# adamjorr/kbbq

Hardware: AMD Instinct MI355X
Metric: recalibrated Gbases/sec (higher is better)
Workload: dtype u64

## Files before the change

kbbq_amd/csrc/bucket.h:

```cpp
#pragma once
#include <hip/hip_runtime.h>
#include <stdint.h>

#include "device_common.h"

namespace kbbq {

constexpr int SUB_BITS = 12;
constexpr int NB2_BITS = 9;
constexpr int SUB_BLOCKS = 1 << SUB_BITS;
constexpr int NB2 = 1 << NB2_BITS;
constexpr int L1_SHIFT = SUB_BITS + NB2_BITS;
constexpr int MAX_NB1 = 512;
constexpr int N_XCD = 8;
constexpr int CNT_STRIDE = 32;
constexpr int BK_THREADS = 512;
constexpr int EMIT_GRID = 512;

struct BucketDev {
    unsigned long long *l1;
    uint32_t *l1_cnt;
    uint32_t *l2;
    uint32_t *l2_cnt;
    uint32_t *tickets;
    unsigned long long *direct;
    uint32_t cap1, cap2;
    int nb1;
    int n_src;
    int cnt_stride;
    uint32_t n_sub;
};

__device__ __forceinline__ int xcc_id() {
    unsigned x;
    asm volatile("s_getreg_b32 %0, hwreg(HW_REG_XCC_ID, 0, 4)" : "=s"(x));
    return (int)(x & (N_XCD - 1));
}

__device__ __forceinline__ uint32_t block_scan512(uint32_t v, uint32_t *wave_tot, uint32_t *total) {
    const int lane = threadIdx.x & 63, w = threadIdx.x >> 6;
    uint32_t inc = v;
#pragma unroll
    for (int o = 1; o < 64; o <<= 1) { const uint32_t y = __shfl_up(inc, o); if (lane >= o) inc += y; }
    if (lane == 63) wave_tot[w] = inc;
    __syncthreads();
    uint32_t before = 0, all = 0;
#pragma unroll
    for (int i = 0; i < 8; ++i) { const uint32_t t = wave_tot[i]; before += i < w ? t : 0; all += t; }
    *total = all;
    return before + inc - v;
}

template <int NW, int CH, bool BY_BASE, int RPW, bool PRIV, bool DENSE = true>
__global__ void __launch_bounds__(BK_THREADS) k_emit_marked(ReadsDev R, KParams K, FiltDev F, BucketDev B, const uint64_t *mask,
                                                             uint64_t mask_words, const uint64_t *kofs,
                                                             unsigned long long *inserted) {
    using S = Stage<NW>;
    constexpr int SLOTS = RPW * CH;
    extern __shared__ unsigned long long sorted[];
    __shared__ uint32_t stage[8][DENSE ? RPW : 1][2 * S::WORDS];
    __shared__ uint32_t hist[MAX_NB1], ofs_l[MAX_NB1], gbase_l[MAX_NB1], fill_l[MAX_NB1], wave_tot[8];
    const int lane = threadIdx.x & 63;
    const int w = __builtin_amdgcn_readfirstlane(threadIdx.x >> 6);
    uint32_t *L32 = stage[w][0];
    const int k = K.k;
    const int src = PRIV ? (int)blockIdx.x : xcc_id();
    const uint64_t reads_per_tile = 8 * RPW;
    const uint64_t n_tiles = (R.n_reads + reads_per_tile - 1) / reads_per_tile;
    unsigned long long mine = 0, direct = 0;
    hist[threadIdx.x] = 0;
    if (PRIV) fill_l[threadIdx.x] = (int)threadIdx.x < B.nb1 ? B.l1_cnt[(size_t)src * B.nb1 + threadIdx.x] : 0u;
    __syncthreads();
    uint64_t off[RPW], kb[RPW], word[RPW];
    uint32_t len[RPW];
    auto fetch_tile = [&](uint64_t tile) {
        const uint64_t r0 = (tile * 8 + w) * RPW;
#pragma unroll
        for (int rr = 0; rr < RPW; ++rr) {
            off[rr] = 0; kb[rr] = 0; word[rr] = 0; len[rr] = 0;
            if (r0 + rr < R.n_reads) {
                read_span(R, r0 + rr, off[rr], len[rr]);
                kb[rr] = BY_BASE ? off[rr] : kmer_base(kofs, r0 + rr, R.read_len, k);
                word[rr] = stage_fetch<NW>(R, nullptr, mask, kb[rr], mask_words - 1, off[rr], lane);
            }
        }
    };
    if (blockIdx.x < n_tiles) fetch_tile(blockIdx.x);
    for (uint64_t tile = blockIdx.x; tile < n_tiles; tile += gridDim.x) {
        unsigned long long rec[SLOTS];
        int rk[SLOTS];
#pragma unroll
        for (int s = 0; s < SLOTS; ++s) { rec[s] = 0; rk[s] = -1; }
        if (DENSE) {
            unsigned long long *wlist = sorted + (size_t)w * SLOTS * 64;
            int n_dense = 0;
            __builtin_amdgcn_wave_barrier();
            if (lane < S::WORDS) {
#pragma unroll
                for (int rr = 0; rr < RPW; ++rr) stage_store(stage[w][rr], lane, word[rr]);
            }
            __builtin_amdgcn_wave_barrier();
#pragma unroll
            for (int rr = 0; rr < RPW; ++rr) {
                const int nk = (int)len[rr] - k + 1;
                if (nk > 0) {
                    const uint32_t *L32 = stage[w][rr];
// ... 27 lines not shown
        } else {
#pragma unroll
        for (int rr = 0; rr < RPW; ++rr) {
            const int nk = (int)len[rr] - k + 1;
            if (nk > 0) {
                __builtin_amdgcn_wave_barrier();
                if (lane < S::WORDS) stage_store(L32, lane, word[rr]);
                __builtin_amdgcn_wave_barrier();
                const int o31 = (int)(off[rr] & 31), o63 = (int)(off[rr] & 63), x63 = (int)(kb[rr] & 63);
#pragma unroll
                for (int c = 0; c < CH; ++c) {
                    if (c * 64 < nk) {
                        const int s = c * 64 + lane;
                        const bool marked = lds_bit(L32 + 2 * S::X, x63 + s) != 0;
                        const bool valid = (lds_window32(L32 + 2 * S::M, o63 + s) & K.nmask_bits) == 0;
                        const bool take = s < nk && marked && (BY_BASE || valid);
                        const uint64_t key = canon_key(lds_window64(L32 + 2 * S::B, 2 * (o31 + s)), K);
                        const uint32_t blk = block_of(F, key);
                        rec[rr * CH + c] = ((unsigned long long)blk << 16) | pattern_of(F, key);
                        if (take) rk[rr * CH + c] = (int)atomicAdd(&hist[blk >> L1_SHIFT], 1u);
                        const unsigned long long bal = __ballot(take);
                        if (!BY_BASE && R.hint_sampled) or_bits64(R.hint_sampled, off[rr] + (uint64_t)c * 64, bal, lane);
                        mine += __popcll(bal);
                    }
                }
            }
        }
        }
        if (tile + gridDim.x < n_tiles) fetch_tile(tile + gridDim.x);
        __syncthreads();
        const uint32_t cnt = hist[threadIdx.x];
        hist[threadIdx.x] = 0;
        uint32_t g = 0;
        if (PRIV) {
            g = fill_l[threadIdx.x];
            fill_l[threadIdx.x] = g + cnt;
        } else if (cnt) {
            g = atomicAdd(&B.l1_cnt[((size_t)src * B.nb1 + threadIdx.x) * CNT_STRIDE], cnt);
        }
        uint32_t total;
        const uint32_t ex = block_scan512(cnt, wave_tot, &total);
        ofs_l[threadIdx.x] = ex;
        gbase_l[threadIdx.x] = g;
        __syncthreads();
#pragma unroll
        for (int s = 0; s < SLOTS; ++s)
            if (rk[s] >= 0) sorted[ofs_l[(uint32_t)(rec[s] >> (16 + L1_SHIFT))] + (uint32_t)rk[s]] = rec[s];
        __syncthreads();
        for (uint32_t i = threadIdx.x; i < total; i += BK_THREADS) {
            const unsigned long long v = sorted[i];
            const uint32_t b = (uint32_t)(v >> (16 + L1_SHIFT));
            const uint32_t pos = gbase_l[b] + (i - ofs_l[b]);
            if (pos < B.cap1) {
                B.l1[((size_t)src * B.nb1 + b) * B.cap1 + pos] = v;
            } else {
                bloom_put(F, (uint32_t)(v >> 16), (uint32_t)(v & 0xFFFFu));
                ++direct;
            }
        }
        if (DENSE) __syncthreads();
    }
    if (PRIV && (int)threadIdx.x < B.nb1) B.l1_cnt[(size_t)src * B.nb1 + threadIdx.x] = fill_l[threadIdx.x];
    if (inserted && lane == 0 && mine) atomicAdd(inserted, mine);
    if (direct) atomicAdd(B.direct, direct);
}

constexpr int SPLIT_PER_THREAD = 12;
constexpr int SPLIT_TILE = BK_THREADS * SPLIT_PER_THREAD;

__global__ void __launch_bounds__(BK_THREADS) k_split(FiltDev F, BucketDev B, uint32_t chunks_per_region) {
    __shared__ uint32_t hist[NB2], ofs_l[NB2], gbase_l[NB2], wave_tot[8], unit_l;
    __shared__ uint32_t sorted[SPLIT_TILE];
    __shared__ uint16_t sorted_b[SPLIT_TILE];
    const int home = xcc_id();
    unsigned long long direct = 0;
    hist[threadIdx.x] = 0;
    for (int qi = 0; qi < N_XCD; ++qi) {
        const int q = (home + qi) & (N_XCD - 1);
        const uint32_t n_buckets = B.nb1 > q ? (uint32_t)(B.nb1 - q + N_XCD - 1) / N_XCD : 0;
        const uint32_t n_units = n_buckets * (uint32_t)B.n_src * chunks_per_region;
        for (;;) {
            __syncthreads();
            if (threadIdx.x == 0) unit_l = atomicAdd(&B.tickets[q * CNT_STRIDE], 1u);
            __syncthreads();
            const uint32_t unit = unit_l;
            if (unit >= n_units) break;
            const uint32_t chunk = unit % chunks_per_region, rest = unit / chunks_per_region;
            const int x = (int)(rest % (uint32_t)B.n_src), b1 = q + (int)(rest / (uint32_t)B.n_src) * N_XCD;
            const size_t region = (size_t)x * B.nb1 + b1;
            const uint32_t n = min(B.l1_cnt[region * B.cnt_stride], B.cap1);
            const uint32_t first = chunk * (uint32_t)SPLIT_TILE;
            if (first >= n) continue;
            const uint32_t m = min((uint32_t)SPLIT_TILE, n - first);
            const unsigned long long *src = B.l1 + region * B.cap1 + first;
            uint32_t rec[SPLIT_PER_THREAD];
            int rk[SPLIT_PER_THREAD];
#pragma unroll
            for (int j = 0; j < SPLIT_PER_THREAD; ++j) {
                const uint32_t i = j * BK_THREADS + threadIdx.x;
                rk[j] = -1;
                rec[j] = 0;
                if (i < m) {
                    const unsigned long long v = src[i];
                    rec[j] = (uint32_t)v;
                    rk[j] = (int)atomicAdd(&hist[(uint32_t)(v >> (16 + SUB_BITS)) & (NB2 - 1)], 1u);
                    rk[j] |= (int)(((uint32_t)(v >> (16 + SUB_BITS)) & (NB2 - 1)) << 16);
                }
            }
            __syncthreads();
            const uint32_t cnt = hist[threadIdx.x];
            hist[threadIdx.x] = 0;
            uint32_t g = 0;
            if (cnt) g = atomicAdd(&B.l2_cnt[(size_t)b1 * NB2 + threadIdx.x], cnt);
            uint32_t total;
            const uint32_t ex = block_scan512(cnt, wave_tot, &total);
            ofs_l[threadIdx.x] = ex;
            gbase_l[threadIdx.x] = g;
            __syncthreads();
#pragma unroll
            for (int j = 0; j < SPLIT_PER_THREAD; ++j)
                if (rk[j] >= 0) {
                    const uint32_t b2 = (uint32_t)rk[j] >> 16, at = ofs_l[b2] + ((uint32_t)rk[j] & 0xFFFFu);
                    sorted[at] = rec[j] & 0x0FFFFFFFu;
                    sorted_b[at] = (uint16_t)b2;
                }
            __syncthreads();
            for (uint32_t i = threadIdx.x; i < total; i += BK_THREADS) {
                const uint32_t v = sorted[i], b2 = sorted_b[i];
                const uint32_t pos = gbase_l[b2] + (i - ofs_l[b2]);
                const size_t sub = (size_t)b1 * NB2 + b2;
                if (pos < B.cap2) {
                    B.l2[sub * B.cap2 + pos] = v;
                } else {
                    bloom_put(F, (uint32_t)(sub << SUB_BITS) | (v >> 16), v & 0xFFFFu);
                    ++direct;
                }
            }
        }
    }
    if (direct) atomicAdd(B.direct, direct);
}

constexpr int APPLY_THREADS = 1024;

__global__ void __launch_bounds__(APPLY_THREADS) k_apply(FiltDev F, BucketDev B) {
    __shared__ ulonglong2 blk_l[SUB_BLOCKS];
    const uint32_t sub = blockIdx.x;
    const uint32_t n = min(B.l2_cnt[sub], B.cap2);
    if (n == 0) return;
    const uint64_t b0 = (uint64_t)sub << SUB_BITS;
    const uint32_t nblk = (uint32_t)min((uint64_t)SUB_BLOCKS, F.n_blocks - b0);
    const uint32_t *src = B.l2 + (size_t)sub * B.cap2;
    const uint32_t last = n - 1;
    uint32_t v[3][4];
    ulonglong2 p[3][4];
#pragma unroll
    for (int s = 0; s < 3; ++s)
#pragma unroll
        for (int j = 0; j < 4; ++j) v[s][j] = src[min(threadIdx.x + (4 * s + j) * APPLY_THREADS, last)];
#pragma unroll
    for (int j = 0; j < 4; ++j) p[0][j] = F.patterns[v[0][j] & 0xFFFFu];
    for (uint32_t i = threadIdx.x; i < nblk; i += APPLY_THREADS) blk_l[i] = F.table[b0 + i];
    __syncthreads();
    unsigned long long *w = reinterpret_cast<unsigned long long *>(blk_l);
    for (uint32_t i1 = threadIdx.x; i1 < n; i1 += 12 * APPLY_THREADS) {
#pragma unroll
        for (int s = 0; s < 3; ++s) {
            const uint32_t i0 = i1 + 4 * s * APPLY_THREADS;
            const int s2 = (s + 1) % 3;
#pragma unroll
            for (int j = 0; j < 4; ++j) p[s2][j] = F.patterns[v[s2][j] & 0xFFFFu];
#pragma unroll
            for (int j = 0; j < 4; ++j) {
                if (i0 + j * APPLY_THREADS < n) {
                    const uint32_t bi = v[s][j] >> 16;
                    const ulonglong2 t = blk_l[bi];
                    const unsigned long long mx = p[s][j].x & ~t.x, my = p[s][j].y & ~t.y;
                    if (mx) atomicOr(&w[2 * bi], mx);
                    if (my) atomicOr(&w[2 * bi + 1], my);
                }
            }
#pragma unroll
            for (int j = 0; j < 4; ++j) v[s][j] = src[min(i0 + (12 + j) * APPLY_THREADS, last)];
        }
    }
    __syncthreads();
    for (uint32_t i = threadIdx.x; i < nblk; i += APPLY_THREADS) F.table[b0 + i] = blk_l[i];
}

}
```

kbbq_amd/csrc/engine.hip:

```cpp
#include <hip/hip_runtime.h>

#include <algorithm>
#include <climits>
#include <cstdarg>
#include <cstdio>
#include <cstdlib>
#include <cstring>
#include <map>
#include <mutex>
#include <string>
#include <thread>
#include <vector>

#include "../../include/kbbq_engine.h"
#include "abi_internal.h"
#include "correct.h"
#include "correct_wave.h"
#include "device_common.h"
#include "host_model.h"

using namespace kbbq;

static thread_local char g_err[512] = "";
int kbbq_fail(int code, const char *fmt, ...) {
// ... 9 lines not shown
        hipError_t _e = (expr);                                                                        \
        if (_e != hipSuccess)                                                                          \
            return fail(_e == hipErrorOutOfMemory ? KBBQ_ENOMEM : KBBQ_EIO, "%s: %s (%s:%d)", #expr,   \
                        hipGetErrorString(_e), __FILE__, __LINE__);                                    \
    } while (0)

#include "kernels.h"
#include "bucket.h"
#include "long_reads.h"


struct FilterHost {
    FilterSpec spec;
    uint64_t *d_table = nullptr;
    uint64_t *d_patterns = nullptr;
    unsigned long long *d_inserted = nullptr;
    uint64_t table_bytes() const { return spec.n_blocks * kEngineBlockBytes; }
    FiltDev dev() const {
        FiltDev f;
        f.table = reinterpret_cast<ulonglong2 *>(d_table);
        f.patterns = reinterpret_cast<const ulonglong2 *>(d_patterns);
        f.n_blocks = spec.n_blocks;
        const ModMagic mm = make_mod_magic(spec.n_blocks);
        f.mod_magic = mm.m64;
        f.mod_m32 = mm.m32;
        f.salt0 = spec.salt[0];
        f.salt1 = spec.salt[1];
        return f;
    }
};

struct ProfileSlot {
    std::string name;
    uint64_t launches = 0;
    double ms = 0;
};
struct PendingEvent {
    int slot;
    hipEvent_t a, b;
};

constexpr int kNoOverride = INT_MIN;
struct Options {
    bool no_overlap = false;
    bool no_fastpath = false;
    bool lane_walk = false;
    bool no_pass4_pipeline = false;
    int pass2_side = 2;
    bool tally_general = false;
    bool infer_subset = true;
    bool debug_bucket = false;
    int bucket = -1;
    uint64_t bucket_records = 0;
    uint64_t pass4_piece = 0;
    int scan_blocks = -1;
    int walk_blocks = -1;
    int infer_blocks = 0;
    int subset_edge = kNoOverride;
    int subset_pmask = kNoOverride;
};


enum Scratch {
    S_KMER_PREFIX,
    S_HOST_OUT,
    S_HOST_FLAGS,
    S_DRAW0, S_DRAW1,
    S_TAKE1,
    S_READ_INDEX0, S_READ_INDEX1,
    S_TMASK, S_DIRTY, S_LIST, S_ERR, S_PATCH,
    S_OFFCASE_LIST,
    S_WALK_WORDS,
    S_SIDE1,
    S_COUNT = S_SIDE1 + (S_SIDE1 - S_TMASK),
    S_TAKE0 = S_ERR + (S_SIDE1 - S_TMASK),
};
constexpr int per_side(Scratch name, int side) { return name + side * (S_SIDE1 - S_TMASK); }

struct SideCounters { unsigned long long list_len, queries; };
struct Counters {
    SideCounters side0;
    unsigned long long kmer_total;
    unsigned long long infer_fetched;
    SideCounters side1;
    unsigned long long offcase_len[2];
    SideCounters *side(int s) { return s ? &side1 : &side0; }
};
struct Tickets {
    unsigned int infer, scan[2], walk[2], unused[11];
};
struct Totals {
    unsigned long long walk_reads, walk_queries;
    unsigned long long digest, unused;
};
static_assert(sizeof(Counters) == 64 && offsetof(Counters, kmer_total) == 16 && offsetof(Counters, side1) == 32 && offsetof(Counters, offcase_len) == 48, "d_counters");
static_assert(sizeof(Tickets) == 64 && offsetof(Tickets, scan) == 4 && offsetof(Tickets, walk) == 12, "d_tickets");
static_assert(sizeof(Totals) == 32 && offsetof(Totals, digest) == 16, "d_totals");

struct Pass3 {
    int side;
    hipStream_t stream;
    int stream_no;
    unsigned long long *cnt;
    unsigned int *scan_ticket, *wave_ticket;
    bool shared;
};
// ... 392 lines not shown

int upload_dq(kbbq_engine *e) {
    const DqTables &d = e->dq;
    const size_t nb = d.n_rg * kNQ, nc = d.n_rg * kNQ * 2 * d.n_cycle, nd = d.n_rg * kNQ * 16;
    std::vector<int16_t> base(nb);
    std::vector<int8_t> cyc(nc), di(nd);
    for (uint64_t r = 0; r < d.n_rg; ++r)
        for (int q = 0; q < kNQ; ++q) base[r * kNQ + q] = (int16_t)(d.meanq[r] + d.rgdq[r] + d.qdq[r * kNQ + q]);
    for (size_t i = 0; i < nc; ++i) cyc[i] = (int8_t)d.cycledq[i];
    for (size_t i = 0; i < nd; ++i) di[i] = (int8_t)d.dinucdq[i];
    HIP_TRY(hipMemcpyAsync(e->d_dq_base, base.data(), nb * 2, hipMemcpyHostToDevice, e->stream));
    HIP_TRY(hipMemcpyAsync(e->d_dq_cycle, cyc.data(), nc, hipMemcpyHostToDevice, e->stream));
    HIP_TRY(hipMemcpyAsync(e->d_dq_dinuc, di.data(), nd, hipMemcpyHostToDevice, e->stream));
    uint8_t slot[KBBQ_NQ];
    memset(slot, 255, sizeof slot);
    int n_slots = 0;
    for (int q = 0; q < kNQ; ++q) {
        bool any = false;
        for (uint64_t r = 0; r < d.n_rg && !any; ++r) {
            const size_t c0 = (r * kNQ + q) * 2 * d.n_cycle, d0 = (r * kNQ + q) * 16;
            for (size_t i = 0; i < 2 * d.n_cycle && !any; ++i) any = cyc[c0 + i] != 0;
            for (size_t i = 0; i < 16 && !any; ++i) any = di[d0 + i] != 0;
        }
        if (any && n_slots < 255) slot[q] = (uint8_t)n_slots;
        if (any) ++n_slots;
    }
    e->dq_slots = n_slots;
    HIP_TRY(hipMemcpyAsync(e->d_dq_qslot, slot, KBBQ_NQ, hipMemcpyHostToDevice, e->stream));
    HIP_TRY(hipStreamSynchronize(e->stream));
    e->dq_set = true;
    return KBBQ_OK;
}

uint64_t env_u64(const char *name, uint64_t dflt) {
    const char *v = getenv(name);
    return v && *v ? strtoull(v, nullptr, 10) : dflt;
}

constexpr bool bucket_private() { return true; }

void bucket_shape(uint64_t n_blocks, uint64_t capacity, uint32_t *n_sub, int *nb1, uint32_t *cap1, uint32_t *cap2) {
    *n_sub = (uint32_t)((n_blocks + SUB_BLOCKS - 1) >> SUB_BITS);
    *nb1 = (int)((*n_sub + NB2 - 1) >> NB2_BITS);
    const double f1 = std::min(1.0, (double)(1ULL << L1_SHIFT) / (double)n_blocks), f2 = std::min(1.0, (double)SUB_BLOCKS / (double)n_blocks);
    const int n_src = bucket_private() ? EMIT_GRID : N_XCD;
    *cap1 = (uint32_t)std::min(4.0e9, (double)capacity * 1.15 * f1 / n_src) + 64;
    *cap2 = (uint32_t)std::min(4.0e9, (double)capacity * 1.25 * f2) + 32;
}

BucketDev bucket_dev(kbbq_engine *e, int w) {
    BucketDev B;
    bucket_shape(e->filt[w].spec.n_blocks, e->bk.capacity, &B.n_sub, &B.nb1, &B.cap1, &B.cap2);
    B.l1 = (unsigned long long *)e->bk.l1;
    B.l2 = (uint32_t *)e->bk.l2;
    B.l1_cnt = e->bk.l1_cnt;
    B.l2_cnt = e->bk.l2_cnt;
    B.tickets = e->bk.tickets;
    B.direct = e->bk.direct;
    B.n_src = bucket_private() ? EMIT_GRID : N_XCD;
    B.cnt_stride = bucket_private() ? 1 : CNT_STRIDE;
    return B;
}

const size_t kL1CntBytes = (size_t)EMIT_GRID * MAX_NB1 * 4, kL2CntBytes = (size_t)MAX_NB1 * NB2 * 4, kTicketBytes = (size_t)N_XCD * CNT_STRIDE * 4;

bool bucket_on(kbbq_engine *e, int w) {
    kbbq_engine::Buckets &b = e->bk;
    if (b.mode[w] >= 0) return b.mode[w] == 1;
    const uint64_t n_blocks = e->filt[w].spec.n_blocks;
    bool want = e->opt.bucket >= 0 ? e->opt.bucket != 0 : e->filt[w].table_bytes() >= (256u << 20);
    if (n_blocks > ((uint64_t)MAX_NB1 << L1_SHIFT)) want = false;
    if (want && !b.allocated) {
        size_t free_b = 0, total_b = 0;
        if (hipMemGetInfo(&free_b, &total_b) != hipSuccess) free_b = 0;
        const uint64_t big = std::max(e->filt[0].spec.n_blocks, e->filt[1].spec.n_blocks);
        uint64_t cap = (uint64_t)((double)free_b * 0.45 / 14.5);
        cap = std::min<uint64_t>(cap, 4000000000ULL);
        cap = std::min<uint64_t>(cap, std::max<uint64_t>(1u << 20, 32 * big));
        if (e->opt.bucket_records) cap = e->opt.bucket_records;
        cap = std::max<uint64_t>(cap, 4096);
        size_t l1_bytes = 0, l2_bytes = 0;
        for (int f = 0; f < 2; ++f) {
            uint32_t n_sub, cap1, cap2; int nb1;
            bucket_shape(e->filt[f].spec.n_blocks, cap, &n_sub, &nb1, &cap1, &cap2);
            l1_bytes = std::max(l1_bytes, (size_t)(bucket_private() ? EMIT_GRID : N_XCD) * nb1 * cap1 * 8);
            l2_bytes = std::max(l2_bytes, (size_t)n_sub * cap2 * 4);
        }
        hipError_t he = hipMalloc(&b.l1, l1_bytes);
        if (he == hipSuccess) he = hipMalloc(&b.l2, l2_bytes);
        if (he == hipSuccess) he = hipMalloc(&b.l1_cnt, kL1CntBytes);
        if (he == hipSuccess) he = hipMalloc(&b.l2_cnt, kL2CntBytes);
        if (he == hipSuccess) he = hipMalloc(&b.tickets, kTicketBytes);
        if (he == hipSuccess) he = hipMalloc(&b.direct, 8);
        if (he == hipSuccess) he = hipMemsetAsync(b.l1_cnt, 0, kL1CntBytes, e->stream);
        if (he == hipSuccess) he = hipMemsetAsync(b.l2_cnt, 0, kL2CntBytes, e->stream);
        if (he == hipSuccess) he = hipMemsetAsync(b.direct, 0, 8, e->stream);
        if (he != hipSuccess) {
            (void)hipGetLastError();
            hipFree(b.l1); hipFree(b.l2); hipFree(b.l1_cnt); hipFree(b.l2_cnt); hipFree(b.tickets); hipFree(b.direct);
            b.l1 = b.l2 = nullptr; b.l1_cnt = b.l2_cnt = b.tickets = nullptr; b.direct = nullptr;
            want = false;
            b.mode[0] = b.mode[1] = 0;
        } else {
            b.allocated = true;
            b.capacity = cap;
        }
    }
    if (b.mode[w] < 0) b.mode[w] = want ? 1 : 0;
    return b.mode[w] == 1;
}

hipStream_t bucket_stream(kbbq_engine *e, int w) { return e->bk.stream[w] ? e->bk.stream[w] : e->stream; }

void bucket_poll_estimate(kbbq_engine *e) {
    kbbq_engine::Buckets &b = e->bk;
    if (!b.est_pending || hipEventQuery(b.ev_est) != hipSuccess) return;
    const unsigned long long now = *b.h_inserted;
    if (b.est_bases > 0 && now >= b.est_prev)
        b.frac_trusted = std::min(1.0, 1.03 * (double)(now - b.est_prev) / (double)b.est_bases + 0.005);
    b.inserted_at_flush[1] = now;
    b.est_pending = false;
    if (e->opt.debug_bucket) fprintf(stderr, "[bucket] inserted %llu (before %llu) over %llu bases -> %.4f trusted inserts per base\n", now,
                       (unsigned long long)b.est_prev, (unsigned long long)b.est_bases, b.frac_trusted);
}

int bucket_flush(kbbq_engine *e, int w, bool barrier = true) {
    kbbq_engine::Buckets &b = e->bk;
    if (!b.pending[w]) return KBBQ_OK;
    const BucketDev B = bucket_dev(e, w);
    const FiltDev F = e->filt[w].dev();
    const hipStream_t emit_st = bucket_stream(e, w);
    hipStream_t st = emit_st;
    int rc;
    if (w == 1 && e->opt.pass2_side == 2 && emit_st != e->stream) {
        st = e->stream;
        if ((rc = run_after(st, emit_st, b.ev_flush))) return rc;
    }
    HIP_TRY(hipMemsetAsync(b.tickets, 0, kTicketBytes, st));
    {
        Timed t(e, w ? "k_split_trusted" : "k_split_sampled", st);
        const uint32_t chunks = (B.cap1 + SPLIT_TILE - 1) / SPLIT_TILE;
        hipLaunchKernelGGL(k_split, dim3(256 * 3), dim3(BK_THREADS), 0, st, F, B, chunks);
        HIP_TRY(hipGetLastError());
    }
    {
        Timed t(e, w ? "k_apply_trusted" : "k_apply_sampled", st);
        hipLaunchKernelGGL(k_apply, dim3(B.n_sub), dim3(APPLY_THREADS), 0, st, F, B);
        HIP_TRY(hipGetLastError());
    }
    HIP_TRY(hipMemsetAsync(b.l1_cnt, 0, kL1CntBytes, st));
    HIP_TRY(hipMemsetAsync(b.l2_cnt, 0, (size_t)B.nb1 * NB2 * 4, st));
    if (st != emit_st && (rc = run_after(emit_st, st, b.ev_flush))) return rc;
    if (st != e->stream && barrier && (rc = run_after(e->stream, st, b.ev_flush))) return rc;
    if (w == 1 && !barrier) {
        bucket_poll_estimate(e);
        if (!b.est_pending && b.h_inserted) {
            HIP_TRY(hipMemcpyAsync(b.h_inserted, e->filt[1].d_inserted, 8, hipMemcpyDeviceToHost, e->stream));
            HIP_TRY(hipEventRecord(b.ev_est, e->stream));
            b.est_pending = true;
            b.est_bases = b.bases_since[1] + b.cur_bases;
            b.est_prev = b.inserted_at_flush[1];
            if (!b.est_known) {
                HIP_TRY(hipEventSynchronize(b.ev_est));
                bucket_poll_estimate(e);
                b.est_known = true;
            }
        }
    }
    if (e->opt.debug_bucket) fprintf(stderr, "[bucket] flush %d of filter %d: estimate %.3g records over %llu bases (%.4f per base), barrier %d\n",
                       (int)b.flushes[w], w, b.pending_est[w], (unsigned long long)b.bases_since[w], w ? b.frac_trusted : 0.0, (int)barrier);
    b.bases_since[w] = 0;
    b.pending[w] = false;
    b.pending_est[w] = 0;
    b.flushes[w] += 1;
    return KBBQ_OK;
}

int bucket_flush_all(kbbq_engine *e) {
    for (int w = 0; w < 2; ++w) {
        int rc = bucket_flush(e, w);
        if (rc) return rc;
    }
    return KBBQ_OK;
}

int settle(kbbq_engine *e) {
    int rc = bucket_flush_all(e);
    return rc ? rc : sync_engine(e);
}

int bucket_reserve(kbbq_engine *e, int w, double est, uint64_t bases) {
    kbbq_engine::Buckets &b = e->bk;
    int rc = bucket_flush(e, 1 - w);
    if (rc) return rc;
    b.cur_bases = bases;
    if (b.pending[w] && b.pending_est[w] + est > 0.93 * (double)b.capacity) {
        if ((rc = bucket_flush(e, w, false))) return rc;
        if (w == 1) est = (est - 4096.0) / std::max(1e-9, b.frac_used) * b.frac_trusted + 4096.0;
    }
    b.cur_bases = 0;
    b.pending[w] = true;
    b.pending_est[w] += est;
    b.bases_since[w] += bases;
    return KBBQ_OK;
}

}


extern "C" {

const char *kbbq_last_error(void) { return g_err; }

int kbbq_engine_create(const kbbq_params *params, kbbq_engine **out) {
    if (!params || !out) return fail(KBBQ_EINVAL, "null argument");
    if (params->k < 1 || params->k > KBBQ_MAX_KMER) return fail(KBBQ_ERANGE, "k must be <= %d and > 0", KBBQ_MAX_KMER);
    if (params->n_rg < 1 || params->n_rg > 65535) return fail(KBBQ_EINVAL, "n_rg must be in 1..65535");
    if (params->max_read_len < 1 || params->max_read_len > KBBQ_MAX_READ_LEN)
        return fail(KBBQ_ERANGE, "max_read_len must be in 1..%d", KBBQ_MAX_READ_LEN);
    int ndev = 0;
    if (hipGetDeviceCount(&ndev) != hipSuccess || ndev == 0) return fail(KBBQ_ENODEV, "no HIP device visible");
    if (params->device < 0 || params->device >= ndev) return fail(KBBQ_ENODEV, "device %d of %d", params->device, ndev);
    DeviceGuard create_guard(params->device);
    HIP_TRY(create_guard.err);
    kbbq_engine *e = new kbbq_engine;
    e->p = *params;
    {
        Options &o = e->opt;
        auto env_set = [](const char *name) { const char *v = getenv(name); return v && *v; };
        auto env_int = [](const char *name, int dflt) { const char *v = getenv(name); return v && *v ? atoi(v) : dflt; };
        const int fl = params->flags;
        o.no_overlap = (fl & KBBQ_F_NO_OVERLAP) || env_set("KBBQ_NO_OVERLAP");
        o.no_fastpath = (fl & KBBQ_F_NO_FASTPATH) || env_set("KBBQ_NO_FASTPATH");
        o.lane_walk = (fl & KBBQ_F_LANE_WALK) || (getenv("KBBQ_CORRECT") && !strcmp(getenv("KBBQ_CORRECT"), "lane"));
        o.no_pass4_pipeline = (fl & KBBQ_F_NO_PASS4_PIPELINE) || env_set("KBBQ_NO_PASS4_PIPELINE");
        o.pass2_side = (fl & KBBQ_F_PASS2_INORDER) ? 0 : env_int("KBBQ_PASS2_SIDE", o.pass2_side);
        o.tally_general = env_set("KBBQ_TALLY_GENERAL");
        o.infer_subset = env_int("KBBQ_INFER_SUBSET", 1) != 0;
        o.debug_bucket = env_set("KBBQ_DEBUG_BUCKET");
        o.bucket = (fl & KBBQ_F_BUCKET_ON) ? 1 : (fl & KBBQ_F_BUCKET_OFF) ? 0 : env_set("KBBQ_BUCKET") ? (env_int("KBBQ_BUCKET", 0) != 0 ? 1 : 0) : -1;
        o.bucket_records = env_u64("KBBQ_BUCKET_RECORDS", 0);
        o.pass4_piece = env_u64("KBBQ_PASS4_PIECE", 0);
        o.scan_blocks = env_int("KBBQ_SCAN_BLOCKS", o.scan_blocks);
        o.walk_blocks = env_int("KBBQ_WALK_BLOCKS", o.walk_blocks);
        o.infer_blocks = env_int("KBBQ_INFER_BLOCKS", o.infer_blocks);
        o.subset_edge = env_int("KBBQ_SUBSET_EDGE", o.subset_edge);
        o.subset_pmask = env_int("KBBQ_SUBSET_PMASK", o.subset_pmask);
    }
    e->K.k = params->k;
    e->K.shift = 2u * (unsigned)(params->k - 1);
    e->K.mask = params->k < 32 ? ((1ULL << (2 * params->k)) - 1) : ~0ULL;
    e->K.nmask_bits = params->k < 32 ? ((1u << params->k) - 1) : 0xFFFFFFFFu;
    const double fprs[2] = {params->fpr_sampled, params->fpr_trusted};
    for (int w = 0; w < 2; ++w) {
        if (!make_filter_spec(params->approx_kmers, fprs[w], params->bloom_seed, e->filt[w].spec)) {
            delete e;
            return fail(KBBQ_EINVAL, "Error: Invalid bloom filter parameters. Adjust parameters and try again.");
        }
    }
    hipError_t he = hipStreamCreateWithFlags(&e->stream, hipStreamNonBlocking);
    if (he == hipSuccess) he = hipStreamCreateWithFlags(&e->stream2, hipStreamNonBlocking);
    if (he == hipSuccess) he = hipStreamCreateWithFlags(&e->copy, hipStreamNonBlocking);
    for (hipEvent_t *ev : engine_events(e))
        if (he == hipSuccess) he = hipEventCreateWithFlags(ev, hipEventDisableTiming);
    if (he == hipSuccess) he = hipHostMalloc((void **)&e->bk.h_inserted, 64, hipHostMallocDefault);
    if (he != hipSuccess) { kbbq_engine_destroy(e); return fail(KBBQ_EIO, "hipStreamCreate: %s", hipGetErrorString(he)); }
#define CREATE_TRY(expr)                                                                           \
    do {                                                                                           \
        hipError_t _e = (expr);                                                                    \
        if (_e != hipSuccess) {                                                                    \
            int code = _e == hipErrorOutOfMemory ? KBBQ_ENOMEM : KBBQ_EIO;                         \
            fail(code, "%s: %s", #expr, hipGetErrorString(_e));                                    \
            kbbq_engine_destroy(e);                                                                \
            return code;                                                                           \
        }                                                                                          \
    } while (0)
    CREATE_TRY(hipMalloc(&e->d_counters, sizeof(Counters)));
    CREATE_TRY(hipMemset(e->d_counters, 0, sizeof(Counters)));
    CREATE_TRY(hipMalloc(&e->d_tickets, sizeof(Tickets)));
    CREATE_TRY(hipMemset(e->d_tickets, 0, sizeof(Tickets)));
    CREATE_TRY(hipMalloc(&e->d_totals, sizeof(Totals)));
    CREATE_TRY(hipMemset(e->d_totals, 0, sizeof(Totals)));
    CREATE_TRY(hipMalloc(&e->d_dq_qslot, KBBQ_NQ));
    CREATE_TRY(hipMalloc(&e->d_qpresent, 32));
    for (int i = 0; i < 2; ++i) CREATE_TRY(hipMalloc(&e->d_rg_present[i], (((size_t)params->n_rg + 31) / 32) * 4 + 4));
    for (int w = 0; w < 2; ++w) {
        FilterHost &f = e->filt[w];
        CREATE_TRY(hipMalloc(&f.d_table, f.table_bytes()));
        CREATE_TRY(hipMalloc(&f.d_patterns, kNumPatterns * kEngineBlockBytes));
        CREATE_TRY(hipMalloc(&f.d_inserted, 8));
        std::vector<uint64_t> packed(kNumPatterns * 2);
        for (uint64_t i = 0; i < kNumPatterns; ++i) {
            if (!squeeze_block(&f.spec.patterns[i * 8], &packed[i * 2])) {
                kbbq_engine_destroy(e);
// ... 61 lines not shown
    if (rc0) return rc0;
    for (int w = 0; w < 2; ++w) {
        HIP_TRY(hipMemsetAsync(e->filt[w].d_table, 0, e->filt[w].table_bytes(), e->stream));
        HIP_TRY(hipMemsetAsync(e->filt[w].d_inserted, 0, 8, e->stream));
    }
    HIP_TRY(hipMemsetAsync(e->d_hist, 0, (e->hist_cycle_words + e->hist_dinuc_words) * 8, e->stream));
    HIP_TRY(hipMemsetAsync(e->d_counters, 0, sizeof(Counters), e->stream));
    HIP_TRY(hipMemsetAsync(e->d_totals, 0, offsetof(Totals, digest), e->stream));
    HIP_TRY(hipMemsetAsync(e->d_qpresent, 0, 32, e->stream));
    memset(e->qpresent, 0, sizeof e->qpresent);
    e->qpresent_known = false;
    if (e->bk.allocated) {
        HIP_TRY(hipMemsetAsync(e->bk.l1_cnt, 0, kL1CntBytes, e->stream));
        HIP_TRY(hipMemsetAsync(e->bk.l2_cnt, 0, kL2CntBytes, e->stream));
        HIP_TRY(hipMemsetAsync(e->bk.direct, 0, 8, e->stream));
    }
    e->bk.est_pending = false;
    e->bk.est_known = false;
    e->bk.frac_trusted = 0.75;
    e->bk.stream[0] = e->bk.stream[1] = nullptr;
    for (int w = 0; w < 2; ++w) { e->bk.pending[w] = false; e->bk.pending_est[w] = 0; e->bk.bases_since[w] = 0; e->bk.inserted_at_flush[w] = 0; e->bk.flushes[w] = 0; }
    e->thresholds_set = false;
    e->dq_set = false;
    memset(e->stats, 0, sizeof e->stats);
    return sync_engine(e);
}

int kbbq_engine_sync(kbbq_engine *e) {
    ENGINE_DEVICE(e);
    return settle(e);
}

void *kbbq_engine_stream(kbbq_engine *e) { return e ? (void *)e->stream : nullptr; }

int kbbq_engine_dims(kbbq_engine *e, uint64_t *n_rg, uint64_t *n_cycle) {
    if (!e) return fail(KBBQ_EINVAL, "null engine");
    if (n_rg) *n_rg = (uint64_t)e->p.n_rg;
    if (n_cycle) *n_cycle = (uint64_t)e->p.max_read_len;
    return KBBQ_OK;
}

int kbbq_engine_tune(kbbq_engine *e, const char *name, uint64_t value) {
    if (!e || !name) return fail(KBBQ_EINVAL, "null argument");
    if (!strcmp(name, "bucket_records")) {
        if (e->bk.allocated) return fail(KBBQ_ESTATE, "the record buffers are allocated already");
        e->opt.bucket_records = value;
    } else if (!strcmp(name, "pass4_piece")) {
        e->opt.pass4_piece = value;
    } else if (!strcmp(name, "scan_blocks") || !strcmp(name, "walk_blocks") || !strcmp(name, "infer_blocks")) {
        if (value > 17) return fail(KBBQ_EINVAL, "%s: 0 (as many as fit) to 16 workgroups per CU, 17 = default", name);
        (name[0] == 's' ? e->opt.scan_blocks : name[0] == 'w' ? e->opt.walk_blocks : e->opt.infer_blocks) = value == 17 ? (name[0] == 'i' ? 0 : -1) : (int)value;
    } else if (!strcmp(name, "infer_subset")) {
        e->opt.infer_subset = value != 0;
    } else if (!strcmp(name, "pass2_side") || !strcmp(name, "no_overlap")) {
        ENGINE_DEVICE(e);
        int rc = settle(e);
        if (rc) return rc;
        if (name[0] == 'p' && value > 2) return fail(KBBQ_EINVAL, "pass2_side: 0, 1 or 2");
        if (name[0] == 'p') e->opt.pass2_side = (int)value; else e->opt.no_overlap = value != 0;
        e->bk.stream[0] = e->bk.stream[1] = nullptr;
    } else {
        return fail(KBBQ_EINVAL, "unknown knob '%s'", name);
    }
    return KBBQ_OK;
}

int kbbq_filter_info_get(kbbq_engine *e, int which, kbbq_filter_info *out) {
    ENGINE_DEVICE(e);
    if (!out || which < 0 || which > 1) return fail(KBBQ_EINVAL, "bad argument");
    int rc = settle(e);
    if (rc) return rc;
    const FilterSpec &s = e->filt[which].spec;
    memset(out, 0, sizeof *out);
    out->bits = s.bits;
    out->bits_unblocked = s.bits_unblocked;
    out->n_blocks = s.n_blocks;
    out->table_bytes = e->filt[which].table_bytes();
    out->random_seed = s.random_seed;
    out->n_hash = s.n_hash;
    out->n_salt = s.n_salt;
    for (uint32_t i = 0; i < s.n_salt; ++i) out->salt[i] = s.salt[i];
    HIP_TRY(hipMemcpy(&out->inserted, e->filt[which].d_inserted, 8, hipMemcpyDeviceToHost));
    return KBBQ_OK;
}

void *kbbq_filter_device_table(kbbq_engine *e, int which) {
    if (!e || which < 0 || which > 1) return nullptr;
    DeviceGuard guard(e->p.device);
    if (guard.err != hipSuccess || bucket_flush_all(e) != KBBQ_OK) return nullptr;
    return e->filt[which].d_table;
}
void *kbbq_filter_device_counter(kbbq_engine *e, int which) { return e && which >= 0 && which < 2 ? e->filt[which].d_inserted : nullptr; }

int kbbq_filter_download(kbbq_engine *e, int which, uint64_t *host_words, uint64_t n_words) {
    ENGINE_DEVICE(e);
    if (!host_words || which < 0 || which > 1) return fail(KBBQ_EINVAL, "bad argument");
    const uint64_t n_blocks = e->filt[which].spec.n_blocks;
    if (n_words != n_blocks * 8) return fail(KBBQ_EINVAL, "filter has %llu words", (unsigned long long)n_blocks * 8);
    int rc = settle(e);
    if (rc) return rc;
    const uint64_t chunk = 1 << 20;
    std::vector<uint64_t> packed(chunk * 2);
    for (uint64_t b0 = 0; b0 < n_blocks; b0 += chunk) {
        const uint64_t nb = std::min(chunk, n_blocks - b0);
        HIP_TRY(hipMemcpy(packed.data(), e->filt[which].d_table + b0 * 2, nb * kEngineBlockBytes, hipMemcpyDeviceToHost));
        for (uint64_t b = 0; b < nb; ++b) expand_block(&packed[b * 2], host_words + (b0 + b) * 8);
// ... 398 lines not shown
int kbbq_device_memory(int32_t device, uint64_t *free_bytes, uint64_t *total_bytes) {
    int cur = 0;
    HIP_TRY(hipGetDevice(&cur));
    if (device >= 0 && device != cur) HIP_TRY(hipSetDevice(device));
    size_t f = 0, t = 0;
    HIP_TRY(hipMemGetInfo(&f, &t));
    if (device >= 0 && device != cur) HIP_TRY(hipSetDevice(cur));
    if (free_bytes) *free_bytes = f;
    if (total_bytes) *total_bytes = t;
    return KBBQ_OK;
}

int kbbq_count_kmer_positions(kbbq_engine *e, const kbbq_reads *reads, uint64_t *out) {
    ENGINE_DEVICE(e);
    if (!reads || !out) return fail(KBBQ_EINVAL, "null argument");
    HostBatchDone host_done(e, reads);
    ReadsDev R; int max_len;
    int rc = device_view(e, reads, &R, &max_len, false);
    if (rc) return rc;
    const uint64_t *kofs;
    return kmer_prefix(e, R, &kofs, out);
}

}

constexpr int kStagedMax = 512;
constexpr int kTallyMaxWindows = 24;
template <template <int> class Launcher, typename... Args>
static int dispatch_nw(int max_len, Args... args) {
    if (max_len <= 192) return Launcher<3>::go(args...);
    if (max_len <= 320) return Launcher<5>::go(args...);
    return Launcher<8>::go(args...);
}

template <int NW> struct LaunchSample {
    static int go(kbbq_engine *e, ReadsDev R, const uint64_t *mask, uint64_t mask_words, const uint64_t *kofs) {
        Timed t(e, "k_insert_sampled");
        hipLaunchKernelGGL((k_insert_marked<NW, false>), dim3(wave_grid(R.n_reads)), dim3(256), 0, e->stream, R, e->K,
                           e->filt[0].dev(), mask, mask_words, kofs, e->filt[0].d_inserted);
        HIP_TRY(hipGetLastError());
        return KBBQ_OK;
    }
};

template <int NW, int CH, int RPW>
static int launch_emit(kbbq_engine *e, int w, ReadsDev R, const uint64_t *mask, uint64_t mask_words, const uint64_t *kofs,
                       unsigned long long *inserted) {
    const BucketDev B = bucket_dev(e, w);
    const uint64_t n_tiles = (R.n_reads + 8 * RPW - 1) / (8 * RPW);
    const int grid = (int)std::min<uint64_t>(n_tiles, EMIT_GRID);
    const size_t lds = (size_t)8 * RPW * CH * 64 * 8;
    hipStream_t st = bucket_stream(e, w);
    Timed t(e, w ? "k_emit_trusted" : "k_emit_sampled", st);
#define KBBQ_EMIT(BYB)                                                                                                        \
    do {                                                                                                                      \
        const void *fn = (const void *)k_emit_marked<NW, CH, BYB, RPW, true, true>;                                            \
        size_t &raised = e->attr_lds_correct[fn];                                                                             \
        if (lds > 48 * 1024 && lds > raised) {                                                                                \
            HIP_TRY(hipFuncSetAttribute(fn, hipFuncAttributeMaxDynamicSharedMemorySize, (int)lds));                            \
            raised = lds;                                                                                                     \
        }                                                                                                                     \
        hipLaunchKernelGGL((k_emit_marked<NW, CH, BYB, RPW, true, true>), dim3(grid), dim3(BK_THREADS), lds, st, R, e->K,      \
                           e->filt[w].dev(), B, mask, mask_words, kofs, inserted);                                            \
    } while (0)
    if (w == 0) KBBQ_EMIT(false); else KBBQ_EMIT(true);
#undef KBBQ_EMIT
    HIP_TRY(hipGetLastError());
    return KBBQ_OK;
}

static int dispatch_emit(kbbq_engine *e, int w, int max_len, ReadsDev R, const uint64_t *mask, uint64_t mask_words, const uint64_t *kofs,
                         unsigned long long *inserted) {
    const int max_nk = std::max(1, max_len - e->p.k + 1);
    if (max_len <= 192) {
        if (max_nk <= 128) return launch_emit<3, 2, 4>(e, w, R, mask, mask_words, kofs, inserted);
        return launch_emit<3, 3, 4>(e, w, R, mask, mask_words, kofs, inserted);
    }
    if (max_len <= 320) return launch_emit<5, 5, 2>(e, w, R, mask, mask_words, kofs, inserted);
    return launch_emit<8, 8, 1>(e, w, R, mask, mask_words, kofs, inserted);
}

extern "C" {

int kbbq_sample_batch(kbbq_engine *e, const kbbq_reads *reads, uint64_t first_kmer_ordinal) {
    ENGINE_DEVICE(e);
    HostBatchDone host_done(e, reads);
    ReadsDev R; int max_len;
    int rc = device_view(e, reads, &R, &max_len, false);
    if (rc) return rc;
    const uint64_t *kofs; uint64_t n_draws;
    if ((rc = kmer_prefix(e, R, &kofs, &n_draws))) return rc;
    if (n_draws == 0) return KBBQ_OK;
    const bool overlap = reads->on_device && !e->opt.no_overlap;
    const int turn = overlap ? e->draw_turn : 0;
    uint64_t *mask;
    if ((rc = scratch_buf(e, turn ? S_DRAW1 : S_DRAW0, (n_draws / 64 + 2) * 8, &mask))) return rc;
    hipStream_t ds = overlap ? e->stream2 : e->stream;
    if (overlap) {
        e->draw_turn ^= 1;
        if (e->ins_pending[turn]) HIP_TRY(hipStreamWaitEvent(ds, e->ev_ins[turn], 0));
    }
    {
        Timed t(e, "k_draw_mask", ds);
        const uint64_t lanes = (n_draws + DRAWS_PER_LANE - 1) / DRAWS_PER_LANE;
        uint64_t st[4];
        xoshiro_state_at(e->p.seed, first_kmer_ordinal, st);
        hipLaunchKernelGGL(k_draw_mask, dim3((unsigned)((lanes + 255) / 256)), dim3(256), 0, ds,
                           st[0], st[1], st[2], st[3],
                           (uint64_t)0, n_draws, e->draw_threshold, e->draw_always ? 1 : 0, mask);
        HIP_TRY(hipGetLastError());
    }
    if (overlap && (rc = run_after(e->stream, ds, e->ev_draw))) return rc;
    if (max_len > kStagedMax) {
        Timed t(e, "k_insert_sampled_long");
        hipLaunchKernelGGL(k_insert_marked_long<false>, dim3(wave_grid(R.n_reads)), dim3(256), 0, e->stream, R, e->K, e->filt[0].dev(),
                           (const uint64_t *)mask, n_draws / 64 + 2, kofs, e->filt[0].d_inserted);
        HIP_TRY(hipGetLastError());
        rc = KBBQ_OK;
// ... 849 lines not shown
```

Before: 24.44.

## Prefetch next split tile and add optional narrow L1 record layout

Restructures k_split so ticket fetch and the global load of the next tile's records overlap with the scatter of the current tile, software-pipelining across loop iterations. It also adds an optional split lo/hi (5-byte) L1 record layout, enabled with KBBQ_L1_WIDE=0, which cuts L1 traffic compared with 8-byte records. Wide records stay the default, so only the prefetching restructure runs by default. The pipelining adds register pressure and more complex control flow.

New measurement: 23.73. 2.9% lower.

```diff
diff --git a/kbbq_amd/csrc/bucket.h b/kbbq_amd/csrc/bucket.h
--- a/kbbq_amd/csrc/bucket.h
+++ b/kbbq_amd/csrc/bucket.h
@@ -18,6 +18,8 @@
 constexpr int EMIT_GRID = 512;
 
 struct BucketDev {
+    uint32_t *l1_lo;
+    uint8_t *l1_hi;
     unsigned long long *l1;
     uint32_t *l1_cnt;
     uint32_t *l2;
@@ -51,7 +53,7 @@
     return before + inc - v;
 }
 
-template <int NW, int CH, bool BY_BASE, int RPW, bool PRIV, bool DENSE = true>
+template <int NW, int CH, bool BY_BASE, int RPW, bool PRIV, bool DENSE = true, bool WIDE = false>
 __global__ void __launch_bounds__(BK_THREADS) k_emit_marked(ReadsDev R, KParams K, FiltDev F, BucketDev B, const uint64_t *mask,
                                                              uint64_t mask_words, const uint64_t *kofs,
                                                              unsigned long long *inserted) {
@@ -185,7 +187,13 @@
             const uint32_t b = (uint32_t)(v >> (16 + L1_SHIFT));
             const uint32_t pos = gbase_l[b] + (i - ofs_l[b]);
             if (pos < B.cap1) {
-                B.l1[((size_t)src * B.nb1 + b) * B.cap1 + pos] = v;
+                const size_t at = ((size_t)src * B.nb1 + b) * B.cap1 + pos;
+                if (WIDE) {
+                    B.l1[at] = v;
+                } else {
+                    B.l1_lo[at] = (uint32_t)v;
+                    B.l1_hi[at] = (uint8_t)((uint32_t)(v >> 32) & 31u);
+                }
             } else {
                 bloom_put(F, (uint32_t)(v >> 16), (uint32_t)(v & 0xFFFFu));
                 ++direct;
@@ -199,65 +207,99 @@
 }
 
 constexpr int SPLIT_PER_THREAD = 12;
+constexpr uint32_t SPLIT_DONE = 0xFFFFFFFFu;
 constexpr int SPLIT_TILE = BK_THREADS * SPLIT_PER_THREAD;
 
+template <bool WIDE>
 __global__ void __launch_bounds__(BK_THREADS) k_split(FiltDev F, BucketDev B, uint32_t chunks_per_region) {
-    __shared__ uint32_t hist[NB2], ofs_l[NB2], gbase_l[NB2], wave_tot[8], unit_l;
-    __shared__ uint32_t sorted[SPLIT_TILE];
-    __shared__ uint16_t sorted_b[SPLIT_TILE];
+    constexpr int SPT = SPLIT_PER_THREAD, TILE = SPLIT_TILE;
+    static_assert(TILE <= 0x10000, "ranks are kept in 16 bits");
+    __shared__ uint32_t hist[NB2], ofs_l[NB2], gbase_l[NB2], wave_tot[8], unit_l[2][4];
+    __shared__ uint32_t sorted[TILE];
+    __shared__ uint16_t sorted_b[TILE];
     const int home = xcc_id();
-    unsigned long long direct = 0;
+    uint32_t direct = 0;
     hist[threadIdx.x] = 0;
-    for (int qi = 0; qi < N_XCD; ++qi) {
-        const int q = (home + qi) & (N_XCD - 1);
-        const uint32_t n_buckets = B.nb1 > q ? (uint32_t)(B.nb1 - q + N_XCD - 1) / N_XCD : 0;
-        const uint32_t n_units = n_buckets * (uint32_t)B.n_src * chunks_per_region;
-        for (;;) {
-            __syncthreads();
-            if (threadIdx.x == 0) unit_l = atomicAdd(&B.tickets[q * CNT_STRIDE], 1u);
-            __syncthreads();
-            const uint32_t unit = unit_l;
-            if (unit >= n_units) break;
-            const uint32_t chunk = unit % chunks_per_region, rest = unit / chunks_per_region;
-            const int x = (int)(rest % (uint32_t)B.n_src), b1 = q + (int)(rest / (uint32_t)B.n_src) * N_XCD;
-            const size_t region = (size_t)x * B.nb1 + b1;
-            const uint32_t n = min(B.l1_cnt[region * B.cnt_stride], B.cap1);
-            const uint32_t first = chunk * (uint32_t)SPLIT_TILE;
-            if (first >= n) continue;
-            const uint32_t m = min((uint32_t)SPLIT_TILE, n - first);
-            const unsigned long long *src = B.l1 + region * B.cap1 + first;
-            uint32_t rec[SPLIT_PER_THREAD];
-            int rk[SPLIT_PER_THREAD];
-#pragma unroll
-            for (int j = 0; j < SPLIT_PER_THREAD; ++j) {
-                const uint32_t i = j * BK_THREADS + threadIdx.x;
-                rk[j] = -1;
-                rec[j] = 0;
-                if (i < m) {
-                    const unsigned long long v = src[i];
-                    rec[j] = (uint32_t)v;
-                    rk[j] = (int)atomicAdd(&hist[(uint32_t)(v >> (16 + SUB_BITS)) & (NB2 - 1)], 1u);
-                    rk[j] |= (int)(((uint32_t)(v >> (16 + SUB_BITS)) & (NB2 - 1)) << 16);
-                }
-            }
-            __syncthreads();
+    int tq = 0;
+    uint32_t ticket = 0;
+    if (threadIdx.x == 0) ticket = atomicAdd(&B.tickets[home * CNT_STRIDE], 1u);
+    uint32_t b1 = 0, m = 0, b1_n = 0, m_n = 0;
+    size_t at_n = 0;
+    uint32_t lo[SPT], hi[SPT];
+#pragma unroll
+    for (int j = 0; j < SPT; ++j) lo[j] = hi[j] = 0;
+    auto load_next = [&]() {
+        if (m_n == 0) return;
+        const uint32_t last = m_n - 1;
+#pragma unroll
+        for (int j = 0; j < SPT; ++j) {
+            const uint32_t i = min(j * BK_THREADS + threadIdx.x, last);
+            if (WIDE) {
+                const unsigned long long v = (B.l1 + at_n)[i];
+                lo[j] = (uint32_t)v;
+                hi[j] = (uint32_t)(v >> 32);
+            } else {
+                lo[j] = (B.l1_lo + at_n)[i];
+                hi[j] = (B.l1_hi + at_n)[i];
+            }
+        }
+    };
+    for (uint32_t it = 0;; ++it) {
+        if (b1 == SPLIT_DONE) break;
+        if (threadIdx.x == 0) {
+            uint32_t pb1 = SPLIT_DONE, pregion = 0, pfirst = 0;
+            while (tq < N_XCD) {
+                const int q = (home + tq) & (N_XCD - 1);
+                const uint32_t n_buckets = B.nb1 > q ? (uint32_t)(B.nb1 - q + N_XCD - 1) / N_XCD : 0;
+                const uint32_t n_units = n_buckets * (uint32_t)B.n_src * chunks_per_region;
+                if (ticket < n_units) {
+                    const uint32_t chunk = ticket % chunks_per_region, rest = ticket / chunks_per_region;
+                    pb1 = (uint32_t)q + (rest / (uint32_t)B.n_src) * N_XCD;
+                    pregion = (rest % (uint32_t)B.n_src) * (uint32_t)B.nb1 + pb1;
+                    pfirst = chunk * (uint32_t)TILE;
+                    break;
+                }
+                if (++tq < N_XCD) ticket = atomicAdd(&B.tickets[((home + tq) & (N_XCD - 1)) * CNT_STRIDE], 1u);
+            }
+            uint32_t *u = unit_l[it & 1];
+            u[0] = pb1; u[1] = pregion; u[2] = pfirst;
+            if (tq < N_XCD) ticket = atomicAdd(&B.tickets[((home + tq) & (N_XCD - 1)) * CNT_STRIDE], 1u);
+        }
+        if (m) {
+#pragma unroll
+            for (int j = 0; j < SPT; ++j) {
+                const uint32_t b2 = ((hi[j] << 4) | (lo[j] >> 28)) & (NB2 - 1);
+                hi[j] = SPLIT_DONE;
+                if (j * BK_THREADS + threadIdx.x < m) hi[j] = atomicAdd(&hist[b2], 1u) | (b2 << 16);
+            }
+        }
+        __syncthreads();
+        const uint32_t *u = unit_l[it & 1];
+        const uint32_t region_v = u[1];
+        const uint32_t b1_f = __builtin_amdgcn_readfirstlane(u[0]), first_f = __builtin_amdgcn_readfirstlane(u[2]);
+        uint32_t n_f = 0;
+        if (b1_f != SPLIT_DONE) n_f = B.l1_cnt[(size_t)region_v * B.cnt_stride];
+        uint32_t total = 0;
+        if (m) {
             const uint32_t cnt = hist[threadIdx.x];
             hist[threadIdx.x] = 0;
             uint32_t g = 0;
             if (cnt) g = atomicAdd(&B.l2_cnt[(size_t)b1 * NB2 + threadIdx.x], cnt);
-            uint32_t total;
             const uint32_t ex = block_scan512(cnt, wave_tot, &total);
             ofs_l[threadIdx.x] = ex;
             gbase_l[threadIdx.x] = g;
             __syncthreads();
 #pragma unroll
-            for (int j = 0; j < SPLIT_PER_THREAD; ++j)
-                if (rk[j] >= 0) {
-                    const uint32_t b2 = (uint32_t)rk[j] >> 16, at = ofs_l[b2] + ((uint32_t)rk[j] & 0xFFFFu);
-                    sorted[at] = rec[j] & 0x0FFFFFFFu;
+            for (int j = 0; j < SPT; ++j)
+                if (hi[j] != SPLIT_DONE) {
+                    const uint32_t b2 = hi[j] >> 16, at = ofs_l[b2] + (hi[j] & 0xFFFFu);
+                    sorted[at] = lo[j] & 0x0FFFFFFFu;
                     sorted_b[at] = (uint16_t)b2;
                 }
             __syncthreads();
+        }
+        load_next();
+        if (m) {
             for (uint32_t i = threadIdx.x; i < total; i += BK_THREADS) {
                 const uint32_t v = sorted[i], b2 = sorted_b[i];
                 const uint32_t pos = gbase_l[b2] + (i - ofs_l[b2]);
@@ -270,8 +312,14 @@
                 }
             }
         }
+        b1 = b1_n;
+        m = m_n;
+        b1_n = b1_f;
+        const uint32_t n = min((uint32_t)__builtin_amdgcn_readfirstlane(n_f), B.cap1);
+        m_n = b1_n != SPLIT_DONE && first_f < n ? min((uint32_t)TILE, n - first_f) : 0u;
+        at_n = (size_t)__builtin_amdgcn_readfirstlane(region_v) * B.cap1 + first_f;
     }
-    if (direct) atomicAdd(B.direct, direct);
+    if (direct) atomicAdd(B.direct, (unsigned long long)direct);
 }
 
 constexpr int APPLY_THREADS = 1024;
diff --git a/kbbq_amd/csrc/engine.hip b/kbbq_amd/csrc/engine.hip
--- a/kbbq_amd/csrc/engine.hip
+++ b/kbbq_amd/csrc/engine.hip
@@ -85,6 +85,7 @@
     bool debug_bucket = false;
     int bucket = -1;
     uint64_t bucket_records = 0;
+    bool l1_wide = true;
     uint64_t pass4_piece = 0;
     int scan_blocks = -1;
     int walk_blocks = -1;
@@ -583,6 +584,8 @@
     BucketDev B;
     bucket_shape(e->filt[w].spec.n_blocks, e->bk.capacity, &B.n_sub, &B.nb1, &B.cap1, &B.cap2);
     B.l1 = (unsigned long long *)e->bk.l1;
+    B.l1_lo = (uint32_t *)e->bk.l1;
+    B.l1_hi = (uint8_t *)e->bk.l1 + (size_t)(bucket_private() ? EMIT_GRID : N_XCD) * B.nb1 * B.cap1 * 4;
     B.l2 = (uint32_t *)e->bk.l2;
     B.l1_cnt = e->bk.l1_cnt;
     B.l2_cnt = e->bk.l2_cnt;
@@ -671,7 +674,8 @@
     {
         Timed t(e, w ? "k_split_trusted" : "k_split_sampled", st);
         const uint32_t chunks = (B.cap1 + SPLIT_TILE - 1) / SPLIT_TILE;
-        hipLaunchKernelGGL(k_split, dim3(256 * 3), dim3(BK_THREADS), 0, st, F, B, chunks);
+        if (e->opt.l1_wide) hipLaunchKernelGGL(k_split<true>, dim3(256 * 3), dim3(BK_THREADS), 0, st, F, B, chunks);
+        else hipLaunchKernelGGL(k_split<false>, dim3(256 * 3), dim3(BK_THREADS), 0, st, F, B, chunks);
         HIP_TRY(hipGetLastError());
     }
     {
@@ -771,6 +775,7 @@
         o.debug_bucket = env_set("KBBQ_DEBUG_BUCKET");
         o.bucket = (fl & KBBQ_F_BUCKET_ON) ? 1 : (fl & KBBQ_F_BUCKET_OFF) ? 0 : env_set("KBBQ_BUCKET") ? (env_int("KBBQ_BUCKET", 0) != 0 ? 1 : 0) : -1;
         o.bucket_records = env_u64("KBBQ_BUCKET_RECORDS", 0);
+        o.l1_wide = env_int("KBBQ_L1_WIDE", 1) != 0;
         o.pass4_piece = env_u64("KBBQ_PASS4_PIECE", 0);
         o.scan_blocks = env_int("KBBQ_SCAN_BLOCKS", o.scan_blocks);
         o.walk_blocks = env_int("KBBQ_WALK_BLOCKS", o.walk_blocks);
@@ -938,6 +943,12 @@
         (name[0] == 's' ? e->opt.scan_blocks : name[0] == 'w' ? e->opt.walk_blocks : e->opt.infer_blocks) = value == 17 ? (name[0] == 'i' ? 0 : -1) : (int)value;
     } else if (!strcmp(name, "infer_subset")) {
         e->opt.infer_subset = value != 0;
+    } else if (!strcmp(name, "l1_wide")) {
+        if (e->bk.pending[0] || e->bk.pending[1]) return fail(KBBQ_ESTATE, "l1_wide: records are pending (kbbq_engine_sync first)");
+        ENGINE_DEVICE(e);
+        int rc = settle(e);
+        if (rc) return rc;
+        e->opt.l1_wide = value != 0;
     } else if (!strcmp(name, "pass2_side") || !strcmp(name, "no_overlap")) {
         ENGINE_DEVICE(e);
         int rc = settle(e);
@@ -1442,18 +1453,19 @@
     const size_t lds = (size_t)8 * RPW * CH * 64 * 8;
     hipStream_t st = bucket_stream(e, w);
     Timed t(e, w ? "k_emit_trusted" : "k_emit_sampled", st);
-#define KBBQ_EMIT(BYB)                                                                                                        \
+#define KBBQ_EMIT(BYB, WIDE)                                                                                                  \
     do {                                                                                                                      \
-        const void *fn = (const void *)k_emit_marked<NW, CH, BYB, RPW, true, true>;                                            \
+        const void *fn = (const void *)k_emit_marked<NW, CH, BYB, RPW, true, true, WIDE>;                                      \
         size_t &raised = e->attr_lds_correct[fn];                                                                             \
         if (lds > 48 * 1024 && lds > raised) {                                                                                \
             HIP_TRY(hipFuncSetAttribute(fn, hipFuncAttributeMaxDynamicSharedMemorySize, (int)lds));                            \
             raised = lds;                                                                                                     \
         }                                                                                                                     \
-        hipLaunchKernelGGL((k_emit_marked<NW, CH, BYB, RPW, true, true>), dim3(grid), dim3(BK_THREADS), lds, st, R, e->K,      \
+        hipLaunchKernelGGL((k_emit_marked<NW, CH, BYB, RPW, true, true, WIDE>), dim3(grid), dim3(BK_THREADS), lds, st, R, e->K, \
                            e->filt[w].dev(), B, mask, mask_words, kofs, inserted);                                            \
     } while (0)
-    if (w == 0) KBBQ_EMIT(false); else KBBQ_EMIT(true);
+    if (e->opt.l1_wide) { if (w == 0) KBBQ_EMIT(false, true); else KBBQ_EMIT(true, true); }
+    else { if (w == 0) KBBQ_EMIT(false, false); else KBBQ_EMIT(true, false); }
 #undef KBBQ_EMIT
     HIP_TRY(hipGetLastError());
     return KBBQ_OK;
```
